# andimarafioti/faster-qwen3-tts

Hardware: AMD Instinct MI355X
Metric: real-time factor (audio s / wall s), Qwen3-TTS-12Hz-0.6B voice-clone streaming chunk_size=8; p50 TTFA in ttfa_ms_p50 (higher is better)
Workload: dtype bf16

## Files before the change

faster-qwen3-tts_amd/csrc/decode_kernels.cuh:

```cuda
#pragma once
#include "fq3_common.cuh"
#include <initializer_list>

namespace fq3 {

enum { PRO_PLAIN = 0, PRO_NORM = 1, PRO_COMBINE = 2 };
enum { EPI_STORE = 0, EPI_RESIDUAL = 1, EPI_SWIGLU = 2 };

constexpr int kHeadDim = 128;
constexpr int kKeysPerTile = 64;
constexpr int kMaxWorkers = 8;
constexpr int kPartStride = kHeadDim + 4;


struct GemvArgs {
    const void* W; int N; int K;
    const void* x;
    const void* norm_w; float eps;
    const void* bias;
    void* y;
    const void* res;
    void* xn_out;
    int up_off;
    const float* part; int n_part; int rep;
// ... 377 lines not shown
#pragma unroll
        for (int w = 0; w < 4; ++w) {
            const float ww = __expf(wm[w][h] - M);
            num = fmaf(ww, wo[w][h][d], num);
            den = fmaf(ww, wl[w][h], den);
        }
        float* p = a.part + (((size_t)g * kMaxWorkers + s) * REP + h) * kPartStride;
        p[d] = num;
        if (d == 0) { p[HD] = M; p[HD + 1] = den; }
    }
}

template <typename T, int REP, bool PAGED>
__global__ __launch_bounds__(256) void attn_decode_kernel(AttnArgs a) { attn_decode_body<T, REP, PAGED>(a); }

template <typename T>
__device__ __forceinline__ void attn_pred_body(const AttnArgs& a, int head) {
    constexpr int HD = kHeadDim;
    const int g = head / a.rep, hh = head - g * a.rep;
    const int lane = threadIdx.x & 63, sub = lane >> 4, c = lane & 15;
    const int pos = a.pos_imm;
    const T* qkv = reinterpret_cast<const T*>(a.qkv);
    const int q_dim = a.n_kv * a.rep * HD, kv_dim = a.n_kv * HD;
    T* kc = reinterpret_cast<T*>(a.kcache) + (size_t)g * a.max_seq * HD;
    T* vc = reinterpret_cast<T*>(a.vcache) + (size_t)g * a.max_seq * HD;
    Raw8<T> qraw, knraw, vnraw, qwraw, kwraw, kr[4], vr[4];
    ldraw<false>(qraw, qkv + (size_t)head * HD + c * 8);
    ldraw<false>(knraw, qkv + q_dim + (size_t)g * HD + c * 8);
    ldraw<false>(vnraw, qkv + q_dim + kv_dim + (size_t)g * HD + c * 8);
    ldraw<false>(qwraw, reinterpret_cast<const T*>(a.q_norm_w) + c * 8);
    ldraw<false>(kwraw, reinterpret_cast<const T*>(a.k_norm_w) + c * 8);
    const f32x4 cs0 = *reinterpret_cast<const f32x4*>(a.cos_row + ((c * 8) & 63)), cs1 = *reinterpret_cast<const f32x4*>(a.cos_row + ((c * 8 + 4) & 63));
    const f32x4 sn0 = *reinterpret_cast<const f32x4*>(a.sin_row + ((c * 8) & 63)), sn1 = *reinterpret_cast<const f32x4*>(a.sin_row + ((c * 8 + 4) & 63));
#pragma unroll
    for (int i = 0; i < 4; ++i) {
        int key = i * 4 + sub;
        key = key < a.max_seq ? key : a.max_seq - 1;
        ldraw<false>(kr[i], kc + (size_t)key * HD + c * 8);
        ldraw<false>(vr[i], vc + (size_t)key * HD + c * 8);
    }
    __builtin_amdgcn_sched_barrier(0);
    const float sgn = c < 8 ? -1.f : 1.f;
    const float cs[8] = {cs0.x, cs0.y, cs0.z, cs0.w, cs1.x, cs1.y, cs1.z, cs1.w};
    const float sn[8] = {sgn * sn0.x, sgn * sn0.y, sgn * sn0.z, sgn * sn0.w, sgn * sn1.x, sgn * sn1.y, sgn * sn1.z, sgn * sn1.w};
    auto norm_rope = [&](const Raw8<T>& raw, const Raw8<T>& wraw, float (&out)[8]) {
#pragma clang fp contract(off)
        float x[8], w[8];
        unpack(raw, x); unpack(wraw, w);
        float ss = 0.f;
#pragma unroll
        for (int i = 0; i < 8; ++i) ss = fmaf(x[i], x[i], ss);
        ss = row16_sum(ss);
        const float rs = 1.0f / sqrtf(ss / (float)HD + a.eps);
#pragma unroll
        for (int i = 0; i < 8; i += 2) {
            float u = x[i] * rs, v = x[i + 1] * rs;
            DT<T>::rnd2(u, v);
            u *= w[i]; v *= w[i + 1];
            DT<T>::rnd2(u, v);
            x[i] = u; x[i + 1] = v;
        }
#pragma unroll
        for (int i = 0; i < 8; i += 2) {
            float a0 = x[i] * cs[i], a1 = x[i + 1] * cs[i + 1];
            float b0 = row16_xor8(x[i]) * sn[i], b1 = row16_xor8(x[i + 1]) * sn[i + 1];
            DT<T>::rnd2(a0, a1); DT<T>::rnd2(b0, b1);
            float r0 = a0 + b0, r1 = a1 + b1;
            DT<T>::rnd2(r0, r1);
            out[i] = r0; out[i + 1] = r1;
        }
    };
    float qr[8], knew[8], vnew[8];
    norm_rope(qraw, qwraw, qr);
    norm_rope(knraw, kwraw, knew);
    unpack(vnraw, vnew);
    if (hh == 0 && sub == 0) {
        DT<T>::st8(kc + (size_t)pos * HD + c * 8, knew);
        DT<T>::st8(vc + (size_t)pos * HD + c * 8, vnew);
    }
    float sc[5];
#pragma unroll
    for (int i = 0; i < 4; ++i) {
        float kf[8], s = 0.f;
        unpack(kr[i], kf);
#pragma unroll
        for (int d = 0; d < 8; ++d) s = fmaf(qr[d], kf[d], s);
        s = row16_sum(s);
        sc[i] = (i * 4 + sub < pos) ? s * a.scale : -INFINITY;
    }
    {
        float s = 0.f;
#pragma unroll
        for (int d = 0; d < 8; ++d) s = fmaf(qr[d], knew[d], s);
        s = row16_sum(s);
        sc[4] = sub == 0 ? s * a.scale : -INFINITY;
    }
    const float mx = wave_max(fmaxf(fmaxf(fmaxf(sc[0], sc[1]), fmaxf(sc[2], sc[3])), sc[4]));
    float p[5], lsum = 0.f, o[8];
#pragma unroll
// ... 116 lines not shown
#pragma unroll
        for (int d = 0; d < 8; ++d) o[d] = p[4] * vnew[d];
#pragma unroll
        for (int i = 0; i < 4; ++i)
#pragma unroll
            for (int d = 0; d < 8; ++d) o[d] = fmaf(p[i], vf[i][d], o[d]);
        const float inv = 1.0f / lsum;
#pragma unroll
        for (int d = 0; d < 8; ++d) o[d] = xrow_sum(o[d]) * inv;
        if (sub == 0) DT<T>::st8(reinterpret_cast<T*>(a.out) + (size_t)(g * REP + h) * HD + c * 8, o);
    }
}

template <typename T>
__global__ __launch_bounds__(64) void attn_pred_kernel(AttnArgs a) { attn_pred_body<T>(a); }

template <typename T>
__global__ __launch_bounds__(256) void rmsnorm_kernel(const T* x, const T* w, T* y, int K, float eps) {
    __shared__ float red[8];
    float ss = 0.f;
    for (int e = threadIdx.x; e < K; e += 256) { const float v = DT<T>::ld(x + e); ss = fmaf(v, v, ss); }
    ss = block_sum<4>(ss, red);
    const float rs = 1.0f / sqrtf(ss / (float)K + eps);
    for (int e = threadIdx.x; e < K; e += 256)
        DT<T>::st(y + e, DT<T>::ld(w + e) * DT<T>::rnd(DT<T>::ld(x + e) * rs));
}

template <typename T>
__global__ void copy_kernel(T* dst, const T* src, int n) {
    const int i = blockIdx.x * blockDim.x + threadIdx.x;
// ... 112 lines not shown
```

faster-qwen3-tts_amd/csrc/fq3_api.hip:

```cpp
#define FQ3_SKINNY_EXTERN
#include "fq3_ctx.h"
#include "sampler.cuh"
#include "sampler_wave.cuh"
#include "skinny_gemm.cuh"

#include <cstdio>
#include <cstdlib>
#include <cstring>
#include <map>
#include <string>
#include <type_traits>
#include <vector>

using namespace fq3;

static thread_local std::string g_err;
static int fail(int code, const std::string& m) { g_err = m; return code; }
int fq3_fail_(int code, const std::string& m) { return fail(code, m); }
#define HIPCHK(x) do { hipError_t e_ = (x); if (e_ != hipSuccess) return fail(FQ3_EHIP, std::string(#x) + ": " + hipGetErrorString(e_)); } while (0)

extern "C" const char* fq3_last_error(void) { return g_err.c_str(); }
extern "C" void fq3_set_error_(const char* msg) { g_err = msg ? msg : ""; }
extern "C" int fq3_abi_version(void) { return FQ3_ABI_VERSION; }

// ... 218 lines not shown
}

extern "C" int fq3_set_option(fq3_ctx* c, const char* key, int value) {
    if (!c || !key) return fail(FQ3_EINVAL, "null argument");
    const std::string k(key);
    if (k == "weight_nt") c->opt_nt = value;
    else if (k == "pred_m2") c->opt_m2 = value;
    else if (k == "pred_attn") c->opt_pred_attn = value;
    else if (k == "rows_per_wave_max") c->opt_rmax = value;
    else if (k == "prefill_mode") c->prefill_mode = value;
    else if (k == "flash_prefill") c->opt_flash_prefill = value;
    else if (k == "flash_small") c->opt_flash_small = value;
    else if (k == "swiglu_tile") c->opt_swiglu_tile = value;
    else if (k == "packed_weights") c->opt_packed = value;
    else if (k == "skinny_gemm") c->opt_no_skinny = !value;
    else return fail(FQ3_EINVAL, "unknown option: " + k);
    fq3_graph_reset(c);
    return FQ3_OK;
}

extern "C" int fq3_graph_reset(fq3_ctx* c) {
    if (!c) return fail(FQ3_EINVAL, "null ctx");
    if (c->exec) { (void)hipGraphExecDestroy(c->exec); c->exec = nullptr; }
    if (c->graph) { (void)hipGraphDestroy(c->graph); c->graph = nullptr; }
    return FQ3_OK;
}

namespace {
struct PackedEntry { void* p; int refs; int N, K; };
std::mutex g_packed_mu;
// ... 44 lines not shown
            if (int r = take(l.o, d.hidden, qd, 0)) return r;
            if (int r = take(l.gate_up, 2 * d.inter, d.hidden, 1)) return r;
            if (int r = take(l.gate_up, 2 * d.inter, d.hidden, 0)) return r;
            if (int r = take(l.down, d.hidden, d.inter, 0)) return r;
        }
        return FQ3_OK;
    };
    if (int r = stack(c->tl, c->cfg.talker)) return r;
    if (int r = stack(c->pl, c->cfg.predictor)) return r;
    for (const fq3_layer_weights& l : c->tl) if (int r = take(l.gate_up, 2 * c->cfg.talker.inter, c->cfg.talker.hidden, 2)) return r;
    if (int r = take(c->wt.codec_head, c->cfg.talker.vocab, c->cfg.talker.hidden, 0)) return r;
    for (const void* h : c->lmh) if (int r = take(h, c->cfg.predictor.vocab, c->cfg.predictor.hidden, 0)) return r;
    return FQ3_OK;
}

extern "C" int fq3_ctx_destroy(fq3_ctx* c) {
    if (!c) return FQ3_OK;
    (void)hipDeviceSynchronize();
    fq3_graph_reset(c);
    packed_release_all(c);
    if (c->cap_stream) (void)hipStreamDestroy(c->cap_stream);
    if (fq3_kv_pool* p = c->tk.pool) {
        (void)fq3_kv_release(c, 0);
        bool last;
        { std::lock_guard<std::mutex> lk(p->mu); last = --p->users == 0; }
        if (p->is_private && last) pool_free_(p);
    }
    for (void* p : c->allocs) (void)hipFree(p);
    delete c;
    return FQ3_OK;
}

extern "C" int fq3_bind_weights(fq3_ctx* c, const fq3_weight_table* w) {
    if (!c || !w) return fail(FQ3_EINVAL, "null argument");
    const int G = c->cfg.num_code_groups;
// ... 4 lines not shown
    if (c->cfg.has_projection && !w->proj_w) return fail(FQ3_EINVAL, "has_projection set but proj_w is null");
    if (w->talker_rope_len < c->cfg.max_seq_len || w->pred_rope_len < G + 1)
        return fail(FQ3_EINVAL, "rope tables shorter than the caches");
    c->wt = *w;
    c->tl.assign(w->talker_layers, w->talker_layers + c->cfg.talker.n_layers);
    c->pl.assign(w->predictor_layers, w->predictor_layers + c->cfg.predictor.n_layers);
    c->pemb.assign(w->predictor_embeddings, w->predictor_embeddings + (G - 1));
    c->lmh.assign(w->lm_heads, w->lm_heads + (G - 1));
    for (auto& l : c->tl) if (!l.qkv || !l.o || !l.gate_up || !l.down || !l.input_norm || !l.post_norm || !l.q_norm || !l.k_norm)
        return fail(FQ3_EINVAL, "talker layer has null weights");
    for (auto& l : c->pl) if (!l.qkv || !l.o || !l.gate_up || !l.down || !l.input_norm || !l.post_norm || !l.q_norm || !l.k_norm)
        return fail(FQ3_EINVAL, "predictor layer has null weights");
    HIPCHK(hipMemcpy(c->d_pemb, c->pemb.data(), (G - 1) * sizeof(void*), hipMemcpyHostToDevice));
    (void)hipDeviceSynchronize();
    packed_release_all(c);
    if (int r = packed_acquire_all(c)) { packed_release_all(c); return r; }
    c->bound = true;
    fq3_graph_reset(c);
    return FQ3_OK;
}

template <typename T, int NCH, int PRO, int EPI, bool NT, int M = 1>
static void launch_gemv_n(const GemvArgs& a, int rmax, hipStream_t s) {
    int R = (a.N + 1023) / 1024;
    if (R > MaxRows<NCH, EPI>::v) R = MaxRows<NCH, EPI>::v;
    if (rmax > 0 && R > rmax) R = rmax;
    if (R < 1) R = 1;
    const int grid = (a.N + 4 * R - 1) / (4 * R);
    const size_t shm = PRO == PRO_COMBINE ? (size_t)M * a.K * sizeof(float) : 0;
    if constexpr (MaxRows<NCH, EPI>::v >= 2) {
        if (R == 2) { hipLaunchKernelGGL((gemv_kernel<T, NCH, PRO, EPI, NT, M, 2>), dim3(grid), dim3(256), shm, s, a); return; }
    }
    hipLaunchKernelGGL((gemv_kernel<T, NCH, PRO, EPI, NT, M, 1>), dim3(grid), dim3(256), shm, s, a);
}
template <typename T, int PRO, int EPI>
static int launch_gemv2_t(const GemvArgs& a, int rmax, hipStream_t s) {
    constexpr int most = PRO == PRO_NORM ? 4 : 6;
    const int n = gemv_chunks(a.K, most);
    if (!n) return fail(FQ3_EUNSUPPORTED, PRO == PRO_NORM ? "code predictor hidden size above 2048" : "code predictor GEMV inner dimension above 3072");
    with_value<1, 2, 4, 6>(n, [&](auto nch) {
        if constexpr (decltype(nch)::value <= most) launch_gemv_n<T, decltype(nch)::value, PRO, EPI, false, 2>(a, rmax, s);
    });
// ... 9 lines not shown
    const int n = gemv_chunks(a.K, most);
    if (!n) return fail(FQ3_EUNSUPPORTED, PRO == PRO_NORM ? "hidden size above 2048" : "GEMV inner dimension above 6144");
    with_value<1, 2, 4, 6, 12>(n, [&](auto nch) {
        if constexpr (decltype(nch)::value <= most) launch_gemv_n<T, decltype(nch)::value, PRO, EPI, NT>(a, rmax, s);
    });
    return 0;
}
template <int PRO, int EPI>
static int launch_gemv(const fq3_ctx* c, const GemvArgs& a, bool nt, hipStream_t s) {
    const int rmax = c->opt_rmax;
    if (c->cfg.dtype == FQ3_BF16)
        return nt ? launch_gemv_t<bf16_t, PRO, EPI, true>(a, rmax, s) : launch_gemv_t<bf16_t, PRO, EPI, false>(a, rmax, s);
    return nt ? launch_gemv_t<float, PRO, EPI, true>(a, rmax, s) : launch_gemv_t<float, PRO, EPI, false>(a, rmax, s);
}

template <typename T, bool PAGED>
static void launch_attn_p(const AttnArgs& a, int rep, int workers, hipStream_t s) {
    with_value<1, 2, 4>(rep, [&](auto r) {
        hipLaunchKernelGGL((attn_decode_kernel<T, decltype(r)::value, PAGED>), dim3(a.n_kv, workers), dim3(256), 0, s, a);
    });
}
template <typename T>
static void launch_attn_t(const AttnArgs& a, int rep, int workers, hipStream_t s) {
    if (a.table) launch_attn_p<T, true>(a, rep, workers, s); else launch_attn_p<T, false>(a, rep, workers, s);
}

struct StepSrc { const void* x0; const int* pos_ptr; int pos_imm; bool kv_only_tail = false; };

static int run_stack(fq3_ctx* c, bool talker, const StepSrc& src, hipStream_t s) {
    const fq3_stack_dims& d = talker ? c->cfg.talker : c->cfg.predictor;
    const std::vector<fq3_layer_weights>& L = talker ? c->tl : c->pl;
    StackBufs& kv = talker ? c->tk : c->pk;
    const int rep = d.n_heads / d.n_kv_heads;
    const int q_dim = d.n_heads * kHeadDim, kv_dim = d.n_kv_heads * kHeadDim;
    const bool nt = c->opt_nt == 2 || (c->opt_nt == 1 && talker);
    const float *cos_row, *sin_row;
    if (src.pos_ptr) { cos_row = c->rope_now; sin_row = c->rope_now + 64; }
    else {
        const int rl = talker ? c->wt.talker_rope_len : c->wt.pred_rope_len;
        int rp = src.pos_imm + (talker ? c->rope_delta : 0);
        rp = rp < 0 ? 0 : (rp >= rl ? rl - 1 : rp);
        cos_row = (talker ? c->wt.talker_cos : c->wt.pred_cos) + (size_t)rp * 64;
        sin_row = (talker ? c->wt.talker_sin : c->wt.pred_sin) + (size_t)rp * 64;
    }
    for (int i = 0; i < d.n_layers; ++i) {
        const fq3_layer_weights& w = L[i];
        const void* xin = i == 0 ? src.x0 : c->h;
        GemvArgs g{};
        g.eps = d.rms_eps;
        g.W = w.qkv; g.N = q_dim + 2 * kv_dim; g.K = d.hidden; g.x = xin;
        g.norm_w = w.input_norm; g.y = c->qkv;
        if (int r = launch_gemv<PRO_NORM, EPI_STORE>(c, g, nt, s)) return r;
        const bool tail_skip = src.kv_only_tail && i == d.n_layers - 1;
        GemvArgs o{};
        o.W = w.o; o.N = d.hidden; o.K = q_dim; o.y = c->h; o.res = xin; o.rep = rep;
        AttnArgs a{};
        a.qkv = c->qkv; a.q_norm_w = w.q_norm; a.k_norm_w = w.k_norm; a.eps = d.rms_eps;
        a.cos_row = cos_row; a.sin_row = sin_row;
        a.kcache = kv.k[i]; a.vcache = kv.v[i]; a.max_seq = kv.max_seq;
        a.table = kv.d_table; a.blk_stride = kv.pool ? (int)kv.pool->blk_elems : 0;
        a.pos_ptr = src.pos_ptr; a.pos_imm = src.pos_imm;
        a.done_ptr = src.pos_ptr ? &c->st->done : nullptr;
        a.n_pad = talker ? c->n_pad : 0;
        a.n_kv = d.n_kv_heads; a.part = c->part;
        a.scale = 1.0f / sqrtf((float)kHeadDim);
        a.rep = rep; a.out = c->attn_out;
        const bool pred_attn = c->opt_pred_attn && !talker && !src.pos_ptr && src.pos_imm <= 16;
// ... 22 lines not shown
}

static int run_predictor_pair(fq3_ctx* c, const void* x_a, const void* x_b, hipStream_t s) {
    const fq3_stack_dims& d = c->cfg.predictor;
    StackBufs& kv = c->pk;
    const int rep = d.n_heads / d.n_kv_heads;
    const int q_dim = d.n_heads * kHeadDim, kv_dim = d.n_kv_heads * kHeadDim;
    for (int i = 0; i < d.n_layers; ++i) {
        const fq3_layer_weights& w = c->pl[i];
        const void* xa = i == 0 ? x_a : c->h;
        const void* xb = i == 0 ? x_b : c->h2;
        GemvArgs g{};
        g.eps = d.rms_eps; g.W = w.qkv; g.N = q_dim + 2 * kv_dim; g.K = d.hidden; g.x = xa; g.x2 = xb;
        g.norm_w = w.input_norm; g.y = c->qkv; g.y2 = c->qkv2;
        if (int r = launch_gemv2<PRO_NORM, EPI_STORE>(c, g, s)) return r;
        for (int m = 0; m < 2; ++m) {
            AttnArgs a{};
            a.qkv = m == 0 ? c->qkv : c->qkv2; a.q_norm_w = w.q_norm; a.k_norm_w = w.k_norm; a.eps = d.rms_eps;
            a.cos_row = c->wt.pred_cos + (size_t)m * 64; a.sin_row = c->wt.pred_sin + (size_t)m * 64;
            a.kcache = kv.k[i]; a.vcache = kv.v[i]; a.max_seq = kv.max_seq;
            a.pos_ptr = nullptr; a.pos_imm = m; a.n_pad = 0; a.n_kv = d.n_kv_heads;
            a.part = c->part + (size_t)m * c->part_stride; a.scale = 1.0f / sqrtf((float)kHeadDim);
            a.rep = rep; a.out = m == 0 ? c->attn_out : c->attn_out2;
            if (c->opt_pred_attn) {
                if (c->cfg.dtype == FQ3_BF16) hipLaunchKernelGGL((attn_pred_kernel<bf16_t>), dim3(d.n_heads), dim3(64), 0, s, a);
                else hipLaunchKernelGGL((attn_pred_kernel<float>), dim3(d.n_heads), dim3(64), 0, s, a);
            } else if (c->cfg.dtype == FQ3_BF16) launch_attn_t<bf16_t>(a, rep, kv.workers, s);
            else launch_attn_t<float>(a, rep, kv.workers, s);
        }
        GemvArgs o{};
        o.W = w.o; o.N = d.hidden; o.K = q_dim; o.y = c->h; o.y2 = c->h2; o.res = xa; o.res2 = xb; o.rep = rep;
        if (c->opt_pred_attn) {
            o.x = c->attn_out; o.x2 = c->attn_out2;
            if (int r = launch_gemv2<PRO_PLAIN, EPI_RESIDUAL>(c, o, s)) return r;
        } else {
            o.part = c->part; o.part_stride2 = c->part_stride; o.n_part = kv.workers;
            if (int r = launch_gemv2<PRO_COMBINE, EPI_RESIDUAL>(c, o, s)) return r;
        }
// ... 248 lines not shown

__global__ void build_seen_kernel(const int64_t* history, int n, unsigned char* seen, int V) {
    for (int i = threadIdx.x; i < V; i += blockDim.x) seen[i] = 0;
    __syncthreads();
    for (int i = threadIdx.x; i < n; i += blockDim.x) { const int id = (int)history[i]; if (id >= 0 && id < V) seen[id] = 1; }
}
template <typename F>
static void dispatch_nc(int V, F&& f) {
    if (V <= 2048) f(std::integral_constant<int, 1>{});
    else f(std::integral_constant<int, 2>{});
}

template <typename T>
static void launch_sample_pred(const DecodeState* st, const T* lg, int V, int cb, const SampleCfg& cfg, const T* nz,
                               int* codes, int G, int64_t* out64, const T* next_emb, T* next_in, int H, bool wave,
                               const TeacherForcing* tf, hipStream_t s) {
    if (wave) dispatch_nc(V, [&](auto nc) {
        constexpr int NC = decltype(nc)::value;
        hipLaunchKernelGGL((sample_pred_wave_kernel<T, NC>), dim3(1), dim3(256), 0, s, st, lg, V, cb, cfg, nz, codes, G,
                           out64, next_emb, next_in, H, tf);
    });
    else hipLaunchKernelGGL((sample_pred_kernel<T>), dim3(1), dim3(256), 0, s, st, lg, V, cb, cfg, nz, codes, G, out64,
                            next_emb, next_in, H, tf);
}
template <typename T>
static void launch_sample_talker(DecodeState* st, const T* lg, int V, const unsigned char* seen, int G, bool wave,
                                 const TeacherForcing* tf, hipStream_t s) {
    if (wave) dispatch_nc(V, [&](auto nc) {
        constexpr int NC = decltype(nc)::value;
        hipLaunchKernelGGL((sample_talker_wave_kernel<T, NC>), dim3(1), dim3(256), 0, s, st, lg, V, seen, G, tf);
    });
    else hipLaunchKernelGGL((sample_talker_kernel<T>), dim3(1), dim3(256), 0, s, st, lg, V, seen, G, tf);
}
template <typename T>
static void launch_sample_api(fq3_ctx* c, const T* lg, int V, const SampleCfg& cfg, const int64_t* history, int n_hist,
                              const T* noise, int64_t* out, hipStream_t s) {
// ... 61 lines not shown

extern "C" int fq3_set_predictor_sampling(fq3_ctx* c, const fq3_sampling* s) {
    if (!c || !s) return fail(FQ3_EINVAL, "null argument");
    if (s->do_sample && !(s->temperature > 0.f)) return fail(FQ3_EINVAL, "temperature must be > 0");
    if ((s->top_p >= 1.0f) != (c->pred_sampling.top_p >= 1.0f)) fq3_graph_reset(c);
    c->pred_sampling = *s;
    return FQ3_OK;
}

template <typename T>
static int predictor_passes_t(fq3_ctx* c, const DecodeState* st_dev, const void* pred_input, const void* noise_imm,
                              int64_t* out64, void* out_logits, hipStream_t s) {
    const fq3_stack_dims &p = c->cfg.predictor, &t = c->cfg.talker;
    const int G = c->cfg.num_code_groups, Vp = p.vocab, Ht = t.hidden;
    SampleCfg scfg = to_cfg(c->pred_sampling);
    for (int pass = 0; pass < G; ++pass) {
        const void* hsrc = c->h;
        if (pass == 0 && c->opt_m2) {
            const T* xa = (const T*)pred_input;
            const T* xb = (const T*)pred_input + Ht;
            if (c->cfg.has_projection) {
                GemvArgs g{};
                g.W = c->wt.proj_w; g.bias = c->wt.proj_b; g.N = p.hidden; g.K = Ht; g.x = xa; g.x2 = xb; g.y = c->pred_x; g.y2 = c->pred_x2;
                if (int r = launch_gemv2<PRO_PLAIN, EPI_STORE>(c, g, s)) return r;
                xa = (const T*)c->pred_x; xb = (const T*)c->pred_x2;
            }
            if (int r = run_predictor_pair(c, xa, xb, s)) return r;
            pass = 1;
            hsrc = c->h2;
        } else {
        const T* x_talker = pass < 2 ? (const T*)pred_input + (size_t)pass * Ht : (const T*)c->pred_next;
        const void* x0 = x_talker;
        if (c->cfg.has_projection) {
            GemvArgs g{};
            g.W = c->wt.proj_w; g.bias = c->wt.proj_b; g.N = p.hidden; g.K = Ht; g.x = x_talker; g.y = c->pred_x;
            if (int r = launch_gemv<PRO_PLAIN, EPI_STORE>(c, g, false, s)) return r;
            x0 = c->pred_x;
        }
        StepSrc src{x0, nullptr, pass};
        src.kv_only_tail = pass == 0;
        if (int r = run_stack(c, false, src, s)) return r;
        }
        if (pass == 0) continue;
        const int cb = pass - 1;
        T* lg = out_logits ? (T*)out_logits + (size_t)cb * Vp : (T*)c->plogits + (size_t)cb * Vp;
        GemvArgs hgm{};
        hgm.eps = p.rms_eps; hgm.W = c->lmh[cb]; hgm.N = Vp; hgm.K = p.hidden; hgm.x = hsrc;
        hgm.norm_w = c->wt.predictor_final_norm; hgm.y = lg;
        if (int r = launch_gemv<PRO_NORM, EPI_STORE>(c, hgm, false, s)) return r;
        const T* nz = noise_imm ? (const T*)noise_imm + (size_t)cb * Vp : nullptr;
        const T* next_emb = cb + 1 < G - 1 ? (const T*)c->pemb[cb] : nullptr;
        launch_sample_pred<T>(st_dev, (const T*)lg, Vp, cb, scfg, nz, st_dev ? c->codes : nullptr, G, out64, next_emb,
                              (T*)c->pred_next, Ht, c->pred_sampling.top_p >= 1.0f, st_dev ? c->tf : nullptr, s);
    }
    return 0;
}

extern "C" int fq3_predictor_loop(fq3_ctx* c, const void* pred_input, const void* noise, int64_t* out_ids,
                                  void* out_logits, void* stream) {
    NEED_BOUND(c);
    if (!pred_input || !out_ids) return fail(FQ3_EINVAL, "null argument");
    if (c->pred_sampling.do_sample && !noise) return fail(FQ3_EINVAL, "predictor sampling enabled but no noise given");
    hipStream_t s = (hipStream_t)stream;
    int r = c->cfg.dtype == FQ3_BF16 ? predictor_passes_t<bf16_t>(c, nullptr, pred_input, noise, out_ids, out_logits, s)
                                     : predictor_passes_t<float>(c, nullptr, pred_input, noise, out_ids, out_logits, s);
    if (r) return r;
    LAUNCH_CHECK();
    return FQ3_OK;
// ... 148 lines not shown
```

faster-qwen3-tts_amd/csrc/fq3_ctx.h:

```cpp
#pragma once
#include "../../include/fq3hip.h"
#include "decode_kernels.cuh"
#include <hip/hip_runtime.h>
#include <mutex>
#include <string>
#include <utility>
#include <vector>

struct fq3_kv_pool {
    int dtype = 0, esz = 2, n_layers = 0, n_kv = 0, n_blocks = 0;
    size_t blk_elems = 0;
    std::vector<void*> k, v;
    std::vector<int> free_list;
    std::mutex mu;
    int in_use_high = 0;
    int users = 0;
    bool is_private = false;
};

struct StackBufs {
    std::vector<void*> k, v;
    int max_seq = 0, workers = 1;
    fq3_kv_pool* pool = nullptr;
    int* d_table = nullptr;
// ... 21 lines not shown
    fq3::DecodeState* st = nullptr;
    fq3::TeacherForcing* tf = nullptr;
    unsigned char* seen = nullptr;
    int* codes = nullptr;
    int64_t* ids64 = nullptr;
    int n_pad = 0, rope_delta = 0;
    int opt_nt = 1;
    int opt_m2 = 1;
    int opt_pred_attn = 1;
    int opt_rmax = 2;
    int opt_flash_prefill = 1;
    int opt_flash_small = 1;
    int opt_swiglu_tile = 1;
    int opt_packed = 1;
    std::vector<std::pair<const void*, int>> packed_refs;
    int opt_no_skinny = 0;
    int prefill_mode = 0;
    bool talker_wave = true;
    fq3_sampling pred_sampling{0.9f, 50, 1.0f, 1, 1.0f};
    hipGraph_t graph = nullptr;
    hipGraphExec_t exec = nullptr;
    hipStream_t cap_stream = nullptr;
    std::vector<void*> allocs;
    fq3_prompt_weights pw{};
    bool pw_bound = false;
    void *pw_x = nullptr, *pw_h = nullptr;
    int pw_cap = 0;
    void* ph_hold = nullptr;
    void *tt_tab = nullptr, *tt_x = nullptr, *tt_h = nullptr;
    int tt_alloc = 0;
// ... 22 lines not shown
```

faster-qwen3-tts_amd/csrc/sampler.cuh:

```cuda
#pragma once
#include "fq3_common.cuh"
#include "decode_kernels.cuh"

namespace fq3 {

constexpr int kMaxVocab = 4096;

__device__ __forceinline__ uint32_t okey(float f) {
    const uint32_t u = __float_as_uint(f);
    return (u & 0x80000000u) ? ~u : (u | 0x80000000u);
}

struct ArgMax { float v; int i; };
__device__ __forceinline__ ArgMax amax2(ArgMax a, ArgMax b) {
    return (b.v > a.v || (b.v == a.v && b.i < a.i)) ? b : a;
}
__device__ __forceinline__ int block_argmax(ArgMax a, float* redv, int* redi) {
#pragma unroll
    for (int o = 32; o > 0; o >>= 1) {
        ArgMax b; b.v = __shfl_xor(a.v, o, 64); b.i = __shfl_xor(a.i, o, 64);
        a = amax2(a, b);
    }
    const int w = threadIdx.x >> 6;
    __syncthreads();
// ... 129 lines not shown
}

template <typename T>
__global__ __launch_bounds__(256) void sample_api_kernel(const T* logits, int V, SampleCfg c, const int64_t* history,
                                                         int n_hist, const T* noise, int64_t* out) {
    __shared__ SampleSmem sm;
    __shared__ unsigned char seen_l[kMaxVocab];
    for (int i = threadIdx.x; i < V; i += 256) { sm.vals[i] = DT<T>::ld(logits + i); seen_l[i] = 0; }
    __syncthreads();
    for (int i = threadIdx.x; i < n_hist; i += 256) { const int id = (int)history[i]; if (id >= 0 && id < V) seen_l[id] = 1; }
    __syncthreads();
    const int tok = sample_core<T>(sm, V, c, n_hist > 0 ? seen_l : nullptr, noise);
    if (threadIdx.x == 0) out[0] = tok;
}

template <typename T>
__global__ __launch_bounds__(256) void sample_pred_kernel(const DecodeState* st, const T* logits, int V, int cb,
                                                          SampleCfg c_imm, const T* noise_imm, int* codes, int G,
                                                          int64_t* out64, const T* next_emb, T* next_in, int H, const TeacherForcing* tf) {
    if (st && st->done) return;
    __shared__ SampleSmem sm;
    __shared__ int s_tok;
    SampleCfg c = c_imm;
    const T* noise = noise_imm;
    int frame = 0;
    if (st) {
        c.temperature = st->p_temperature; c.top_k = st->p_top_k; c.top_p = st->p_top_p; c.do_sample = st->p_do_sample;
        frame = st->frame;
        if (st->pred_noise)
            noise = gptr(reinterpret_cast<const T*>(st->pred_noise)) + ((size_t)(frame % st->noise_frames) * (G - 1) + cb) * V;
    }
    for (int i = threadIdx.x; i < V; i += 256) sm.vals[i] = DT<T>::ld(logits + i);
    __syncthreads();
    int tok = sample_core<T>(sm, V, c, nullptr, noise);
    if (st) tok = forced_or(tf, frame * G + 1 + cb, tok);
    if (threadIdx.x == 0) {
        if (codes) codes[(size_t)frame * G + 1 + cb] = tok;
        if (out64) out64[cb] = tok;
    }
    if (next_emb)
        for (int e = threadIdx.x; e < H; e += 256) next_in[e] = next_emb[(size_t)tok * H + e];
}

template <typename T>
__global__ __launch_bounds__(256) void sample_talker_kernel(DecodeState* st, const T* logits, int V,
                                                            const unsigned char* seen, int G, const TeacherForcing* tf) {
    if (st->done) return;
    __shared__ SampleSmem sm;
    SampleCfg c;
    c.temperature = st->t_temperature; c.top_k = st->t_top_k; c.top_p = st->t_top_p; c.do_sample = st->t_do_sample;
    c.rep_penalty = st->t_rep_penalty;
    c.sup_lo = st->sup_lo; c.sup_hi = st->sup_hi; c.keep_id = st->eos_id;
    const int frame = st->frame;
    c.sup_extra = (frame + 1 < st->min_new) ? st->eos_id : -1;
    const T* noise = st->talker_noise
        ? gptr(reinterpret_cast<const T*>(st->talker_noise)) + (size_t)(frame % st->noise_frames) * V : nullptr;
// ... 12 lines not shown
```

faster-qwen3-tts_amd/csrc/sampler_wave.cuh:

```cuda
#pragma once
#include "sampler.cuh"

namespace fq3 {

__device__ __forceinline__ ArgMax wave_argmax(ArgMax a) {
    ArgMax r;
    r.v = wave_max(a.v);
    r.i = wave_min_i32(a.v == r.v ? a.i : 0x7fffffff);
    return r;
}

struct BlkSmem { int cnt[2][4]; float f[4]; float av[4]; int ai[4]; };

__device__ __forceinline__ float blk_max4(float v, BlkSmem& sm) {
    v = wave_max(v);
    __syncthreads();
    if ((threadIdx.x & 63) == 0) sm.f[threadIdx.x >> 6] = v;
    __syncthreads();
    return fmaxf(fmaxf(sm.f[0], sm.f[1]), fmaxf(sm.f[2], sm.f[3]));
}
__device__ __forceinline__ float blk_sum4(float v, BlkSmem& sm) {
    v = wave_sum(v);
    __syncthreads();
    if ((threadIdx.x & 63) == 0) sm.f[threadIdx.x >> 6] = v;
// ... 139 lines not shown
#pragma unroll
        for (int i = 0; i < 8; ++i) {
            const int id = j * 2048 + threadIdx.x * 8 + i;
            if (id < V) big.vals[id] = f[i];
        }
    }
    __syncthreads();
    const int tok = sample_core<T>(big, V, c, seen, noise);
    __syncthreads();
    return tok;
}

template <typename T, int NC, bool NUCLEUS = false>
__device__ __forceinline__ void sample_pred_wave_body(const DecodeState* st, const T* logits, int V, int cb,
                                                      const SampleCfg& c_imm, const T* noise_imm, int* codes, int G,
                                                      int64_t* out64, const T* next_emb, T* next_in, int H, const TeacherForcing* tf = nullptr) {
    __shared__ BlkSmem sm;
    Raw8<T> xraw[NC];
    issue_logits<T, NC>(xraw, logits, V);
    SampleCfg c = c_imm;
    const T* noise = noise_imm;
    int frame = 0;
    if (st) {
        if (st->done) return;
        c.temperature = st->p_temperature; c.top_k = st->p_top_k; c.top_p = st->p_top_p; c.do_sample = st->p_do_sample;
        frame = st->frame;
        if (st->pred_noise)
            noise = gptr(reinterpret_cast<const T*>(st->pred_noise)) + ((size_t)(frame % st->noise_frames) * (G - 1) + cb) * V;
    }
    int tok;
    if constexpr (NUCLEUS) {
        __shared__ SampleSmem big;
        if (c.do_sample && c.top_p < 1.0f) tok = sample_nucleus_from_regs<T, NC>(xraw, V, c, nullptr, noise, big);
        else tok = sample_wave_core<T, NC>(xraw, V, c, nullptr, noise, sm);
    } else {
        tok = sample_wave_core<T, NC>(xraw, V, c, nullptr, noise, sm);
    }
    if (st) tok = forced_or(tf, frame * G + 1 + cb, tok);
    if (threadIdx.x == 0) {
        if (codes) codes[(size_t)frame * G + 1 + cb] = tok;
        if (out64) out64[cb] = tok;
    }
    if (next_emb) {
        const T* src = next_emb + (size_t)tok * H;
        for (int e = threadIdx.x * 8; e < H; e += 256 * 8) {
            Raw8<T> r; ldraw<false>(r, src + e);
            if (sizeof(T) == 2) *reinterpret_cast<u32x4*>(reinterpret_cast<char*>(next_in) + (size_t)e * 2) = *reinterpret_cast<u32x4*>(&r);
            else { float f[8]; unpack(r, f);
#pragma unroll
                   for (int i = 0; i < 8; ++i) DT<T>::st(next_in + e + i, f[i]); }
        }
    }
}

template <typename T, int NC>
__global__ __launch_bounds__(256) void sample_pred_wave_kernel(const DecodeState* st, const T* logits, int V, int cb,
                                                              SampleCfg c_imm, const T* noise_imm, int* codes, int G,
                                                              int64_t* out64, const T* next_emb, T* next_in, int H, const TeacherForcing* tf) {
    sample_pred_wave_body<T, NC>(st, logits, V, cb, c_imm, noise_imm, codes, G, out64, next_emb, next_in, H, tf);
}

template <typename T, int NC, bool NUCLEUS = false>
__device__ __forceinline__ void sample_talker_wave_body(DecodeState* st, const T* logits, int V, const unsigned char* seen, int G,
                                                        const TeacherForcing* tf = nullptr) {
    __shared__ BlkSmem sm;
    Raw8<T> xraw[NC];
    issue_logits<T, NC>(xraw, logits, V);
    if (st->done) return;
    SampleCfg c;
    c.temperature = st->t_temperature; c.top_k = st->t_top_k; c.top_p = st->t_top_p; c.do_sample = st->t_do_sample;
    c.rep_penalty = st->t_rep_penalty;
    c.sup_lo = st->sup_lo; c.sup_hi = st->sup_hi; c.keep_id = st->eos_id;
    const int frame = st->frame;
    c.sup_extra = (frame + 1 < st->min_new) ? st->eos_id : -1;
// ... 21 lines not shown
```

Baseline: 36.98.

## Precompute predictor layer-0 QKV per codebook token and add paired attention kernel

At bind time, builds a table per code predictor codebook that holds each vocabulary token's embedding already projected, normed and run through the layer-0 QKV matrix. The sampler then copies the chosen token's row straight into the qkv and pred_x buffers. This lets predictor passes from the third onward skip the projection GEMV and the first QKV GEMV. The change also adds an opt-in kernel that launches both two-token prefill attention heads in one grid, off by default. The table costs extra device memory (vocab × qkv width per codebook) and bind-time work, and the sampler kernels now move more data.

```diff
diff --git a/faster-qwen3-tts_amd/csrc/decode_kernels.cuh b/faster-qwen3-tts_amd/csrc/decode_kernels.cuh
--- a/faster-qwen3-tts_amd/csrc/decode_kernels.cuh
+++ b/faster-qwen3-tts_amd/csrc/decode_kernels.cuh
@@ -415,8 +415,9 @@
 template <typename T, int REP, bool PAGED>
 __global__ __launch_bounds__(256) void attn_decode_kernel(AttnArgs a) { attn_decode_body<T, REP, PAGED>(a); }
 
-template <typename T>
-__device__ __forceinline__ void attn_pred_body(const AttnArgs& a, int head) {
+template <typename T, bool PAIR_B = false>
+__device__ __forceinline__ void attn_pred_body(const AttnArgs& a, int head, const T* qkv_a = nullptr, const float* cos_a = nullptr,
+                                               const float* sin_a = nullptr) {
     constexpr int HD = kHeadDim;
     const int g = head / a.rep, hh = head - g * a.rep;
     const int lane = threadIdx.x & 63, sub = lane >> 4, c = lane & 15;
@@ -433,18 +434,29 @@
     ldraw<false>(kwraw, reinterpret_cast<const T*>(a.k_norm_w) + c * 8);
     const f32x4 cs0 = *reinterpret_cast<const f32x4*>(a.cos_row + ((c * 8) & 63)), cs1 = *reinterpret_cast<const f32x4*>(a.cos_row + ((c * 8 + 4) & 63));
     const f32x4 sn0 = *reinterpret_cast<const f32x4*>(a.sin_row + ((c * 8) & 63)), sn1 = *reinterpret_cast<const f32x4*>(a.sin_row + ((c * 8 + 4) & 63));
-#pragma unroll
-    for (int i = 0; i < 4; ++i) {
-        int key = i * 4 + sub;
-        key = key < a.max_seq ? key : a.max_seq - 1;
-        ldraw<false>(kr[i], kc + (size_t)key * HD + c * 8);
-        ldraw<false>(vr[i], vc + (size_t)key * HD + c * 8);
+    Raw8<T> karaw;
+    f32x4 ca0, ca1, sa0, sa1;
+    if constexpr (PAIR_B) {
+        ldraw<false>(karaw, qkv_a + q_dim + (size_t)g * HD + c * 8);
+        ldraw<false>(vr[0], qkv_a + q_dim + kv_dim + (size_t)g * HD + c * 8);
+        ca0 = *reinterpret_cast<const f32x4*>(cos_a + ((c * 8) & 63)); ca1 = *reinterpret_cast<const f32x4*>(cos_a + ((c * 8 + 4) & 63));
+        sa0 = *reinterpret_cast<const f32x4*>(sin_a + ((c * 8) & 63)); sa1 = *reinterpret_cast<const f32x4*>(sin_a + ((c * 8 + 4) & 63));
+#pragma unroll
+        for (int i = 1; i < 4; ++i) zero(vr[i]);
+    } else {
+#pragma unroll
+        for (int i = 0; i < 4; ++i) {
+            int key = i * 4 + sub;
+            key = key < a.max_seq ? key : a.max_seq - 1;
+            ldraw<false>(kr[i], kc + (size_t)key * HD + c * 8);
+            ldraw<false>(vr[i], vc + (size_t)key * HD + c * 8);
+        }
     }
     __builtin_amdgcn_sched_barrier(0);
     const float sgn = c < 8 ? -1.f : 1.f;
     const float cs[8] = {cs0.x, cs0.y, cs0.z, cs0.w, cs1.x, cs1.y, cs1.z, cs1.w};
     const float sn[8] = {sgn * sn0.x, sgn * sn0.y, sgn * sn0.z, sgn * sn0.w, sgn * sn1.x, sgn * sn1.y, sgn * sn1.z, sgn * sn1.w};
-    auto norm_rope = [&](const Raw8<T>& raw, const Raw8<T>& wraw, float (&out)[8]) {
+    auto norm_rope = [&](const Raw8<T>& raw, const Raw8<T>& wraw, const float (&cs)[8], const float (&sn)[8], float (&out)[8]) {
 #pragma clang fp contract(off)
         float x[8], w[8];
         unpack(raw, x); unpack(wraw, w);
@@ -472,9 +484,15 @@
         }
     };
     float qr[8], knew[8], vnew[8];
-    norm_rope(qraw, qwraw, qr);
-    norm_rope(knraw, kwraw, knew);
+    norm_rope(qraw, qwraw, cs, sn, qr);
+    norm_rope(knraw, kwraw, cs, sn, knew);
     unpack(vnraw, vnew);
+    float ka[8] = {0.f, 0.f, 0.f, 0.f, 0.f, 0.f, 0.f, 0.f};
+    if constexpr (PAIR_B) {
+        const float csa[8] = {ca0.x, ca0.y, ca0.z, ca0.w, ca1.x, ca1.y, ca1.z, ca1.w};
+        const float sna[8] = {sgn * sa0.x, sgn * sa0.y, sgn * sa0.z, sgn * sa0.w, sgn * sa1.x, sgn * sa1.y, sgn * sa1.z, sgn * sa1.w};
+        norm_rope(karaw, kwraw, csa, sna, ka);
+    }
     if (hh == 0 && sub == 0) {
         DT<T>::st8(kc + (size_t)pos * HD + c * 8, knew);
         DT<T>::st8(vc + (size_t)pos * HD + c * 8, vnew);
@@ -483,7 +501,10 @@
 #pragma unroll
     for (int i = 0; i < 4; ++i) {
         float kf[8], s = 0.f;
-        unpack(kr[i], kf);
+        if constexpr (PAIR_B) {
+#pragma unroll
+            for (int d = 0; d < 8; ++d) kf[d] = i == 0 ? ka[d] : 0.f;
+        } else unpack(kr[i], kf);
 #pragma unroll
         for (int d = 0; d < 8; ++d) s = fmaf(qr[d], kf[d], s);
         s = row16_sum(s);
@@ -630,6 +651,11 @@
 
 template <typename T>
 __global__ __launch_bounds__(64) void attn_pred_kernel(AttnArgs a) { attn_pred_body<T>(a); }
+template <typename T>
+__global__ __launch_bounds__(64) void attn_pred_pair_kernel(AttnArgs a, AttnArgs b) {
+    if (blockIdx.y == 0) attn_pred_body<T>(a, (int)blockIdx.x);
+    else attn_pred_body<T, true>(b, (int)blockIdx.x, reinterpret_cast<const T*>(a.qkv), a.cos_row, a.sin_row);
+}
 
 template <typename T>
 __global__ __launch_bounds__(256) void rmsnorm_kernel(const T* x, const T* w, T* y, int K, float eps) {
diff --git a/faster-qwen3-tts_amd/csrc/fq3_api.hip b/faster-qwen3-tts_amd/csrc/fq3_api.hip
--- a/faster-qwen3-tts_amd/csrc/fq3_api.hip
+++ b/faster-qwen3-tts_amd/csrc/fq3_api.hip
@@ -256,6 +256,8 @@
     else if (k == "swiglu_tile") c->opt_swiglu_tile = value;
     else if (k == "packed_weights") c->opt_packed = value;
     else if (k == "skinny_gemm") c->opt_no_skinny = !value;
+    else if (k == "pred_pair_attn") c->opt_pred_pair_attn = value;
+    else if (k == "pred_qkv_table") c->opt_pred_qkv_table = value;
     else return fail(FQ3_EINVAL, "unknown option: " + k);
     fq3_graph_reset(c);
     return FQ3_OK;
@@ -330,11 +332,15 @@
     return FQ3_OK;
 }
 
+static void predtab_release_all(fq3_ctx* c);
+static void predtab_acquire_all(fq3_ctx* c);
+
 extern "C" int fq3_ctx_destroy(fq3_ctx* c) {
     if (!c) return FQ3_OK;
     (void)hipDeviceSynchronize();
     fq3_graph_reset(c);
     packed_release_all(c);
+    predtab_release_all(c);
     if (c->cap_stream) (void)hipStreamDestroy(c->cap_stream);
     if (fq3_kv_pool* p = c->tk.pool) {
         (void)fq3_kv_release(c, 0);
@@ -369,18 +375,24 @@
     HIPCHK(hipMemcpy(c->d_pemb, c->pemb.data(), (G - 1) * sizeof(void*), hipMemcpyHostToDevice));
     (void)hipDeviceSynchronize();
     packed_release_all(c);
+    predtab_release_all(c);
     if (int r = packed_acquire_all(c)) { packed_release_all(c); return r; }
+    predtab_acquire_all(c);
     c->bound = true;
     fq3_graph_reset(c);
     return FQ3_OK;
 }
 
+template <int NCH, int EPI>
+static int gemv_rows_per_wave(int N, int rmax) {
+    int R = (N + 1023) / 1024;
+    if (R > MaxRows<NCH, EPI>::v) R = MaxRows<NCH, EPI>::v;
+    if (rmax > 0 && R > rmax) R = rmax;
+    return R < 1 ? 1 : R;
+}
 template <typename T, int NCH, int PRO, int EPI, bool NT, int M = 1>
 static void launch_gemv_n(const GemvArgs& a, int rmax, hipStream_t s) {
-    int R = (a.N + 1023) / 1024;
-    if (R > MaxRows<NCH, EPI>::v) R = MaxRows<NCH, EPI>::v;
-    if (rmax > 0 && R > rmax) R = rmax;
-    if (R < 1) R = 1;
+    const int R = gemv_rows_per_wave<NCH, EPI>(a.N, rmax);
     const int grid = (a.N + 4 * R - 1) / (4 * R);
     const size_t shm = PRO == PRO_COMBINE ? (size_t)M * a.K * sizeof(float) : 0;
     if constexpr (MaxRows<NCH, EPI>::v >= 2) {
@@ -420,6 +432,94 @@
     return nt ? launch_gemv_t<float, PRO, EPI, true>(a, rmax, s) : launch_gemv_t<float, PRO, EPI, false>(a, rmax, s);
 }
 
+template <typename T, int NCH, int PRO, int R>
+__global__ __launch_bounds__(256) void gemv_rows_kernel(GemvArgs a, int x_stride, int y_stride) {
+    a.x = reinterpret_cast<const T*>(a.x) + (size_t)blockIdx.y * x_stride;
+    a.y = reinterpret_cast<T*>(a.y) + (size_t)blockIdx.y * y_stride;
+    gemv_body<T, NCH, PRO, EPI_STORE, false, 1, R>(a);
+}
+template <typename T, int PRO>
+static bool launch_gemv_rows(const GemvArgs& a, int rows, int x_stride, int rmax, hipStream_t s) {
+    const int n = gemv_chunks(a.K, 4);
+    if (!n || rows < 1 || rows > 65535) return false;
+    with_value<1, 2, 4>(n, [&](auto nch) {
+        constexpr int NCH = decltype(nch)::value;
+        const int R = gemv_rows_per_wave<NCH, EPI_STORE>(a.N, rmax);
+        const dim3 grid((a.N + 4 * R - 1) / (4 * R), rows);
+        if (R == 2) hipLaunchKernelGGL((gemv_rows_kernel<T, NCH, PRO, 2>), grid, dim3(256), 0, s, a, x_stride, a.N);
+        else hipLaunchKernelGGL((gemv_rows_kernel<T, NCH, PRO, 1>), grid, dim3(256), 0, s, a, x_stride, a.N);
+    });
+    return true;
+}
+
+namespace {
+struct PredTabEntry { void* qkv0; void* x0; int refs; };
+std::map<std::pair<const void*, const void*>, PredTabEntry> g_predtab;
+}
+template <typename T>
+static bool predtab_build(const fq3_ctx* c, const void* emb, PredTabEntry& e) {
+    const fq3_stack_dims &p = c->cfg.predictor, &t = c->cfg.talker;
+    const int N = (p.n_heads + 2 * p.n_kv_heads) * kHeadDim, V = p.vocab;
+    e = PredTabEntry{nullptr, nullptr, 1};
+    (void)hipGetLastError();
+    bool ok = hipMalloc(&e.qkv0, (size_t)V * N * sizeof(T)) == hipSuccess;
+    if (ok && c->cfg.has_projection) ok = hipMalloc(&e.x0, (size_t)V * p.hidden * sizeof(T)) == hipSuccess;
+    const void* x = emb;
+    if (ok && c->cfg.has_projection) {
+        GemvArgs g{};
+        g.W = c->wt.proj_w; g.bias = c->wt.proj_b; g.N = p.hidden; g.K = t.hidden; g.x = emb; g.y = e.x0;
+        ok = launch_gemv_rows<T, PRO_PLAIN>(g, V, t.hidden, c->opt_rmax, nullptr);
+        x = e.x0;
+    }
+    if (ok) {
+        GemvArgs g{};
+        g.eps = p.rms_eps; g.W = c->pl[0].qkv; g.N = N; g.K = p.hidden; g.x = x; g.norm_w = c->pl[0].input_norm; g.y = e.qkv0;
+        ok = launch_gemv_rows<T, PRO_NORM>(g, V, p.hidden, c->opt_rmax, nullptr);
+    }
+    if (ok) ok = hipGetLastError() == hipSuccess && hipStreamSynchronize(nullptr) == hipSuccess;
+    if (!ok) {
+        (void)hipGetLastError();
+        if (e.qkv0) (void)hipFree(e.qkv0);
+        if (e.x0) (void)hipFree(e.x0);
+    }
+    return ok;
+}
+static void predtab_release_all(fq3_ctx* c) {
+    std::lock_guard<std::mutex> lk(g_packed_mu);
+    for (auto& k : c->predtab_refs) {
+        auto it = g_predtab.find(k);
+        if (it == g_predtab.end() || --it->second.refs > 0) continue;
+        (void)hipFree(it->second.qkv0);
+        if (it->second.x0) (void)hipFree(it->second.x0);
+        g_predtab.erase(it);
+    }
+    c->predtab_refs.clear(); c->pqkv0.clear(); c->px0.clear();
+}
+static void predtab_acquire_all(fq3_ctx* c) {
+    const fq3_stack_dims &p = c->cfg.predictor;
+    const int n_tab = c->cfg.num_code_groups - 2;
+    if (!c->cfg.has_projection && p.hidden != c->cfg.talker.hidden) return;
+    bool ok = true;
+    {
+        std::lock_guard<std::mutex> lk(g_packed_mu);
+        for (int cb = 0; cb < n_tab && ok; ++cb) {
+            const std::pair<const void*, const void*> key{c->pemb[cb], c->pl[0].qkv};
+            auto it = g_predtab.find(key);
+            if (it != g_predtab.end()) ++it->second.refs;
+            else {
+                PredTabEntry e{};
+                ok = c->cfg.dtype == FQ3_BF16 ? predtab_build<bf16_t>(c, c->pemb[cb], e) : predtab_build<float>(c, c->pemb[cb], e);
+                if (!ok) break;
+                it = g_predtab.emplace(key, e).first;
+            }
+            c->predtab_refs.push_back(key);
+            c->pqkv0.push_back(it->second.qkv0);
+            if (c->cfg.has_projection) c->px0.push_back(it->second.x0);
+        }
+    }
+    if (!ok) predtab_release_all(c);
+}
+
 template <typename T, bool PAGED>
 static void launch_attn_p(const AttnArgs& a, int rep, int workers, hipStream_t s) {
     with_value<1, 2, 4>(rep, [&](auto r) {
@@ -431,7 +531,7 @@
     if (a.table) launch_attn_p<T, true>(a, rep, workers, s); else launch_attn_p<T, false>(a, rep, workers, s);
 }
 
-struct StepSrc { const void* x0; const int* pos_ptr; int pos_imm; bool kv_only_tail = false; };
+struct StepSrc { const void* x0; const int* pos_ptr; int pos_imm; bool kv_only_tail = false; bool qkv_ready = false; };
 
 static int run_stack(fq3_ctx* c, bool talker, const StepSrc& src, hipStream_t s) {
     const fq3_stack_dims& d = talker ? c->cfg.talker : c->cfg.predictor;
@@ -456,7 +556,8 @@
         g.eps = d.rms_eps;
         g.W = w.qkv; g.N = q_dim + 2 * kv_dim; g.K = d.hidden; g.x = xin;
         g.norm_w = w.input_norm; g.y = c->qkv;
-        if (int r = launch_gemv<PRO_NORM, EPI_STORE>(c, g, nt, s)) return r;
+        if (!(i == 0 && src.qkv_ready))
+            if (int r = launch_gemv<PRO_NORM, EPI_STORE>(c, g, nt, s)) return r;
         const bool tail_skip = src.kv_only_tail && i == d.n_layers - 1;
         GemvArgs o{};
         o.W = w.o; o.N = d.hidden; o.K = q_dim; o.y = c->h; o.res = xin; o.rep = rep;
@@ -509,6 +610,7 @@
         g.eps = d.rms_eps; g.W = w.qkv; g.N = q_dim + 2 * kv_dim; g.K = d.hidden; g.x = xa; g.x2 = xb;
         g.norm_w = w.input_norm; g.y = c->qkv; g.y2 = c->qkv2;
         if (int r = launch_gemv2<PRO_NORM, EPI_STORE>(c, g, s)) return r;
+        AttnArgs at[2];
         for (int m = 0; m < 2; ++m) {
             AttnArgs a{};
             a.qkv = m == 0 ? c->qkv : c->qkv2; a.q_norm_w = w.q_norm; a.k_norm_w = w.k_norm; a.eps = d.rms_eps;
@@ -517,6 +619,13 @@
             a.pos_ptr = nullptr; a.pos_imm = m; a.n_pad = 0; a.n_kv = d.n_kv_heads;
             a.part = c->part + (size_t)m * c->part_stride; a.scale = 1.0f / sqrtf((float)kHeadDim);
             a.rep = rep; a.out = m == 0 ? c->attn_out : c->attn_out2;
+            at[m] = a;
+        }
+        if (c->opt_pred_attn && c->opt_pred_pair_attn) {
+            if (c->cfg.dtype == FQ3_BF16) hipLaunchKernelGGL((attn_pred_pair_kernel<bf16_t>), dim3(d.n_heads, 2), dim3(64), 0, s, at[0], at[1]);
+            else hipLaunchKernelGGL((attn_pred_pair_kernel<float>), dim3(d.n_heads, 2), dim3(64), 0, s, at[0], at[1]);
+        } else for (int m = 0; m < 2; ++m) {
+            const AttnArgs& a = at[m];
             if (c->opt_pred_attn) {
                 if (c->cfg.dtype == FQ3_BF16) hipLaunchKernelGGL((attn_pred_kernel<bf16_t>), dim3(d.n_heads), dim3(64), 0, s, a);
                 else hipLaunchKernelGGL((attn_pred_kernel<float>), dim3(d.n_heads), dim3(64), 0, s, a);
@@ -795,12 +904,16 @@
 template <typename T>
 static void launch_sample_pred(const DecodeState* st, const T* lg, int V, int cb, const SampleCfg& cfg, const T* nz,
                                int* codes, int G, int64_t* out64, const T* next_emb, T* next_in, int H, bool wave,
-                               const TeacherForcing* tf, hipStream_t s) {
+                               const TeacherForcing* tf, const PredRowTab& tab, hipStream_t s) {
     if (wave) dispatch_nc(V, [&](auto nc) {
         constexpr int NC = decltype(nc)::value;
-        hipLaunchKernelGGL((sample_pred_wave_kernel<T, NC>), dim3(1), dim3(256), 0, s, st, lg, V, cb, cfg, nz, codes, G,
-                           out64, next_emb, next_in, H, tf);
+        if (tab.qkv0) hipLaunchKernelGGL((sample_pred_wave_tab_kernel<T, NC>), dim3(1), dim3(256), 0, s, st, lg, V, cb, cfg, nz, codes, G,
+                                         out64, next_emb, next_in, H, tf, tab);
+        else hipLaunchKernelGGL((sample_pred_wave_kernel<T, NC>), dim3(1), dim3(256), 0, s, st, lg, V, cb, cfg, nz, codes, G,
+                                out64, next_emb, next_in, H, tf);
     });
+    else if (tab.qkv0) hipLaunchKernelGGL((sample_pred_tab_kernel<T>), dim3(1), dim3(256), 0, s, st, lg, V, cb, cfg, nz, codes, G, out64,
+                                          next_emb, next_in, H, tf, tab);
     else hipLaunchKernelGGL((sample_pred_kernel<T>), dim3(1), dim3(256), 0, s, st, lg, V, cb, cfg, nz, codes, G, out64,
                             next_emb, next_in, H, tf);
 }
@@ -892,6 +1005,8 @@
     const fq3_stack_dims &p = c->cfg.predictor, &t = c->cfg.talker;
     const int G = c->cfg.num_code_groups, Vp = p.vocab, Ht = t.hidden;
     SampleCfg scfg = to_cfg(c->pred_sampling);
+    const bool tabs = c->opt_pred_qkv_table && !c->pqkv0.empty();
+    const int qkv_n = (p.n_heads + 2 * p.n_kv_heads) * kHeadDim;
     for (int pass = 0; pass < G; ++pass) {
         const void* hsrc = c->h;
         if (pass == 0 && c->opt_m2) {
@@ -909,14 +1024,18 @@
         } else {
         const T* x_talker = pass < 2 ? (const T*)pred_input + (size_t)pass * Ht : (const T*)c->pred_next;
         const void* x0 = x_talker;
+        const bool ready = tabs && pass >= 2;
         if (c->cfg.has_projection) {
-            GemvArgs g{};
-            g.W = c->wt.proj_w; g.bias = c->wt.proj_b; g.N = p.hidden; g.K = Ht; g.x = x_talker; g.y = c->pred_x;
-            if (int r = launch_gemv<PRO_PLAIN, EPI_STORE>(c, g, false, s)) return r;
+            if (!ready) {
+                GemvArgs g{};
+                g.W = c->wt.proj_w; g.bias = c->wt.proj_b; g.N = p.hidden; g.K = Ht; g.x = x_talker; g.y = c->pred_x;
+                if (int r = launch_gemv<PRO_PLAIN, EPI_STORE>(c, g, false, s)) return r;
+            }
             x0 = c->pred_x;
         }
         StepSrc src{x0, nullptr, pass};
         src.kv_only_tail = pass == 0;
+        src.qkv_ready = ready;
         if (int r = run_stack(c, false, src, s)) return r;
         }
         if (pass == 0) continue;
@@ -928,8 +1047,13 @@
         if (int r = launch_gemv<PRO_NORM, EPI_STORE>(c, hgm, false, s)) return r;
         const T* nz = noise_imm ? (const T*)noise_imm + (size_t)cb * Vp : nullptr;
         const T* next_emb = cb + 1 < G - 1 ? (const T*)c->pemb[cb] : nullptr;
+        PredRowTab tab{};
+        if (tabs && next_emb) {
+            tab.qkv0 = c->pqkv0[cb]; tab.qkv_out = c->qkv; tab.qkv_n16 = (int)((size_t)qkv_n * sizeof(T) / 16);
+            if (!c->px0.empty()) { tab.x0 = c->px0[cb]; tab.x_out = c->pred_x; tab.x_n16 = (int)((size_t)p.hidden * sizeof(T) / 16); }
+        }
         launch_sample_pred<T>(st_dev, (const T*)lg, Vp, cb, scfg, nz, st_dev ? c->codes : nullptr, G, out64, next_emb,
-                              (T*)c->pred_next, Ht, c->pred_sampling.top_p >= 1.0f, st_dev ? c->tf : nullptr, s);
+                              (T*)c->pred_next, Ht, c->pred_sampling.top_p >= 1.0f, st_dev ? c->tf : nullptr, tab, s);
     }
     return 0;
 }
diff --git a/faster-qwen3-tts_amd/csrc/fq3_ctx.h b/faster-qwen3-tts_amd/csrc/fq3_ctx.h
--- a/faster-qwen3-tts_amd/csrc/fq3_ctx.h
+++ b/faster-qwen3-tts_amd/csrc/fq3_ctx.h
@@ -59,6 +59,10 @@
     int opt_swiglu_tile = 1;
     int opt_packed = 1;
     std::vector<std::pair<const void*, int>> packed_refs;
+    int opt_pred_pair_attn = 0;
+    int opt_pred_qkv_table = 1;
+    std::vector<std::pair<const void*, const void*>> predtab_refs;
+    std::vector<const void*> pqkv0, px0;
     int opt_no_skinny = 0;
     int prefill_mode = 0;
     bool talker_wave = true;
diff --git a/faster-qwen3-tts_amd/csrc/sampler.cuh b/faster-qwen3-tts_amd/csrc/sampler.cuh
--- a/faster-qwen3-tts_amd/csrc/sampler.cuh
+++ b/faster-qwen3-tts_amd/csrc/sampler.cuh
@@ -167,10 +167,30 @@
     if (threadIdx.x == 0) out[0] = tok;
 }
 
-template <typename T>
-__global__ __launch_bounds__(256) void sample_pred_kernel(const DecodeState* st, const T* logits, int V, int cb,
-                                                          SampleCfg c_imm, const T* noise_imm, int* codes, int G,
-                                                          int64_t* out64, const T* next_emb, T* next_in, int H, const TeacherForcing* tf) {
+struct PredRowTab {
+    const void* qkv0; void* qkv_out; int qkv_n16;
+    const void* x0; void* x_out; int x_n16;
+};
+__device__ __forceinline__ void tab_row_load(u32x4 (&r)[4], const void* tab, int tok, int n16) {
+    if (!tab) return;
+    const u32x4* src = reinterpret_cast<const u32x4*>(tab) + (size_t)tok * n16;
+#pragma unroll
+    for (int j = 0; j < 4; ++j) { const int i = j * 256 + (int)threadIdx.x; r[j] = src[i < n16 ? i : 0]; }
+}
+__device__ __forceinline__ void tab_row_store(const u32x4 (&r)[4], const void* tab, void* out, int tok, int n16) {
+    if (!tab) return;
+    u32x4* dst = reinterpret_cast<u32x4*>(out);
+#pragma unroll
+    for (int j = 0; j < 4; ++j) { const int i = j * 256 + (int)threadIdx.x; if (i < n16) dst[i] = r[j]; }
+    const u32x4* src = reinterpret_cast<const u32x4*>(tab) + (size_t)tok * n16;
+    for (int i = 1024 + (int)threadIdx.x; i < n16; i += 256) dst[i] = src[i];
+}
+
+template <typename T>
+__device__ __forceinline__ void sample_pred_body(const DecodeState* st, const T* logits, int V, int cb,
+                                                 const SampleCfg& c_imm, const T* noise_imm, int* codes, int G,
+                                                 int64_t* out64, const T* next_emb, T* next_in, int H, const TeacherForcing* tf,
+                                                 const PredRowTab& tab) {
     if (st && st->done) return;
     __shared__ SampleSmem sm;
     __shared__ int s_tok;
@@ -191,8 +211,26 @@
         if (codes) codes[(size_t)frame * G + 1 + cb] = tok;
         if (out64) out64[cb] = tok;
     }
+    u32x4 rq[4], rx[4];
+    tab_row_load(rq, tab.qkv0, tok, tab.qkv_n16);
+    tab_row_load(rx, tab.x0, tok, tab.x_n16);
     if (next_emb)
         for (int e = threadIdx.x; e < H; e += 256) next_in[e] = next_emb[(size_t)tok * H + e];
+    tab_row_store(rq, tab.qkv0, tab.qkv_out, tok, tab.qkv_n16);
+    tab_row_store(rx, tab.x0, tab.x_out, tok, tab.x_n16);
+}
+template <typename T>
+__global__ __launch_bounds__(256) void sample_pred_kernel(const DecodeState* st, const T* logits, int V, int cb,
+                                                          SampleCfg c_imm, const T* noise_imm, int* codes, int G,
+                                                          int64_t* out64, const T* next_emb, T* next_in, int H, const TeacherForcing* tf) {
+    sample_pred_body<T>(st, logits, V, cb, c_imm, noise_imm, codes, G, out64, next_emb, next_in, H, tf, PredRowTab{});
+}
+template <typename T>
+__global__ __launch_bounds__(256) void sample_pred_tab_kernel(const DecodeState* st, const T* logits, int V, int cb,
+                                                              SampleCfg c_imm, const T* noise_imm, int* codes, int G,
+                                                              int64_t* out64, const T* next_emb, T* next_in, int H, const TeacherForcing* tf,
+                                                              PredRowTab tab) {
+    sample_pred_body<T>(st, logits, V, cb, c_imm, noise_imm, codes, G, out64, next_emb, next_in, H, tf, tab);
 }
 
 template <typename T>
diff --git a/faster-qwen3-tts_amd/csrc/sampler_wave.cuh b/faster-qwen3-tts_amd/csrc/sampler_wave.cuh
--- a/faster-qwen3-tts_amd/csrc/sampler_wave.cuh
+++ b/faster-qwen3-tts_amd/csrc/sampler_wave.cuh
@@ -177,7 +177,8 @@
 template <typename T, int NC, bool NUCLEUS = false>
 __device__ __forceinline__ void sample_pred_wave_body(const DecodeState* st, const T* logits, int V, int cb,
                                                       const SampleCfg& c_imm, const T* noise_imm, int* codes, int G,
-                                                      int64_t* out64, const T* next_emb, T* next_in, int H, const TeacherForcing* tf = nullptr) {
+                                                      int64_t* out64, const T* next_emb, T* next_in, int H, const TeacherForcing* tf = nullptr,
+                                                      const PredRowTab& tab = PredRowTab{}) {
     __shared__ BlkSmem sm;
     Raw8<T> xraw[NC];
     issue_logits<T, NC>(xraw, logits, V);
@@ -204,6 +205,9 @@
         if (codes) codes[(size_t)frame * G + 1 + cb] = tok;
         if (out64) out64[cb] = tok;
     }
+    u32x4 rq[4], rx[4];
+    tab_row_load(rq, tab.qkv0, tok, tab.qkv_n16);
+    tab_row_load(rx, tab.x0, tok, tab.x_n16);
     if (next_emb) {
         const T* src = next_emb + (size_t)tok * H;
         for (int e = threadIdx.x * 8; e < H; e += 256 * 8) {
@@ -214,6 +218,8 @@
                    for (int i = 0; i < 8; ++i) DT<T>::st(next_in + e + i, f[i]); }
         }
     }
+    tab_row_store(rq, tab.qkv0, tab.qkv_out, tok, tab.qkv_n16);
+    tab_row_store(rx, tab.x0, tab.x_out, tok, tab.x_n16);
 }
 
 template <typename T, int NC>
@@ -221,6 +227,13 @@
                                                               SampleCfg c_imm, const T* noise_imm, int* codes, int G,
                                                               int64_t* out64, const T* next_emb, T* next_in, int H, const TeacherForcing* tf) {
     sample_pred_wave_body<T, NC>(st, logits, V, cb, c_imm, noise_imm, codes, G, out64, next_emb, next_in, H, tf);
+}
+template <typename T, int NC>
+__global__ __launch_bounds__(256) void sample_pred_wave_tab_kernel(const DecodeState* st, const T* logits, int V, int cb,
+                                                                  SampleCfg c_imm, const T* noise_imm, int* codes, int G,
+                                                                  int64_t* out64, const T* next_emb, T* next_in, int H, const TeacherForcing* tf,
+                                                                  PredRowTab tab) {
+    sample_pred_wave_body<T, NC>(st, logits, V, cb, c_imm, noise_imm, codes, G, out64, next_emb, next_in, H, tf, tab);
 }
 
 template <typename T, int NC, bool NUCLEUS = false>
```

After: 37.77 (median of 6 runs). +2.1%, better.
